# adamchang2000/DenseFusion

Measured on AMD Instinct MI355X. Metric: poses/sec (node) YCB-Video 1000 pts + 2 refine iters, higher is better.
Workload: dtype f32

## Files before the change

densefusion_amd/csrc/split_gemm.hip:

```cpp
#include "igemm.h"
#ifdef DF_DEV
#include <map>
#include <mutex>
#include <tuple>
#endif

namespace df {
namespace {

typedef __bf16 bf16x8 __attribute__((ext_vector_type(8)));
typedef __bf16 bf16x2 __attribute__((ext_vector_type(2)));
typedef float f32x16 __attribute__((ext_vector_type(16)));
typedef float f32x2 __attribute__((ext_vector_type(2)));

constexpr int SBM = 128, SBN = 128, SBK = 32;
constexpr int PLANE_BYTES = 128 * 64;

__device__ __forceinline__ void cut3(float a0, float a1, unsigned &hi, unsigned &mid, unsigned &lo) {
  const bf16x2 h = __builtin_convertvector(f32x2{a0, a1}, bf16x2);
  hi = __builtin_bit_cast(unsigned, h);
  const float r0 = a0 - __builtin_bit_cast(float, hi << 16), r1 = a1 - __builtin_bit_cast(float, hi & 0xFFFF0000u);
  const bf16x2 m = __builtin_convertvector(f32x2{r0, r1}, bf16x2);
  mid = __builtin_bit_cast(unsigned, m);
  const float s0 = r0 - __builtin_bit_cast(float, mid << 16), s1 = r1 - __builtin_bit_cast(float, mid & 0xFFFF0000u);
  const bf16x2 l = __builtin_convertvector(f32x2{s0, s1}, bf16x2);
  lo = __builtin_bit_cast(unsigned, l);
}

__global__ void cut_planes_kernel(const float *__restrict__ w, __bf16 *__restrict__ planes, long elems, long stride) {
  const long i = (long)blockIdx.x * blockDim.x + threadIdx.x;
  if (i >= elems) return;
  unsigned h, m, l;
  cut3(w[i], 0.f, h, m, l);
  unsigned short *pl = reinterpret_cast<unsigned short *>(planes);
  pl[i] = (unsigned short)h; pl[stride + i] = (unsigned short)m; pl[2 * stride + i] = (unsigned short)l;
}

struct SplitArgs {
  const float *in; const __bf16 *wpl; const float *bias; const float *res; const float *prelu; float *out; float *colsum;
  long M, wplane;
  int N, K, in_ld, in_coff, out_ld, out_coff, res_ld, res_coff, act, rows_per_group, rows_valid, bias_group_ld;
  long z_in_coff, z_wgt, z_bias, z_out_coff;
  int tiles_m, tiles_n;
  long cs_rows;
};

__device__ __forceinline__ int piece(int row, int slot) { return row * 64 + ((slot ^ ((row >> 2) & 3)) << 4); }

__device__ __forceinline__ void split_epilogue(const SplitArgs &a, const f32x16 (&acc)[2][2], int z, long row0, int wrow, int nb, int fr, int fh, long cs_row) {
  const float slope = a.act == ACT_PRELU ? a.prelu[0] : 0.f;
  float *out = a.out + z * a.z_out_coff + a.out_coff;
  const float *bias = a.bias ? a.bias + z * a.z_bias : nullptr;
  const float *gbias = bias && a.bias_group_ld > 0 ? bias + (row0 / a.rows_per_group) * a.bias_group_ld : nullptr;
  const int grp = a.rows_per_group > 0 ? (int)(row0 / a.rows_per_group) : 0;
  const long left = a.M - row0;
  const int valid = a.rows_per_group > 0 ? a.rows_valid - (int)(row0 - (long)grp * a.rows_per_group) : (1 << 30);
  const int limit = (int)(left < valid ? left : valid);
#pragma unroll
  for (int j = 0; j < 2; ++j) {
    const int n = nb + j * 32 + fr;
    const float b1 = gbias ? gbias[n] : bias ? bias[n] : 0.f;
    float csum = 0.f;
#pragma unroll
    for (int i = 0; i < 2; ++i) {
      const int tb = wrow + i * 32 + 4 * fh;
      const long mb = row0 + tb;
      float r[16];
      if (a.res) {
#pragma unroll
        for (int e = 0; e < 16; ++e) {
          long m = mb + (e & 3) + 8 * (e >> 2);
          m = m < a.M ? m : a.M - 1;
          r[e] = a.res[m * a.res_ld + a.res_coff + n];
        }
      }
#pragma unroll
      for (int e = 0; e < 16; ++e) {
        const int tr = tb + (e & 3) + 8 * (e >> 2);
        const long m = row0 + tr;
        float v = acc[i][j][e] + b1;
        if (a.res) v += r[e];
        if (a.act == ACT_RELU) v = v > 0.f ? v : 0.f;
        else if (a.act == ACT_PRELU) v = v > 0.f ? v : v * slope;
        if (a.out && m < a.M) out[m * a.out_ld + n] = v;
        csum += tr < limit ? v : 0.f;
      }
    }
    if (a.colsum && cs_row < a.cs_rows) {
      csum += __shfl_xor(csum, 32);
      if (fh == 0) a.colsum[((size_t)z * a.cs_rows + (size_t)cs_row) * a.N + n] = csum;
    }
  }
}

__global__ __launch_bounds__(256, 2) void gemm_split_bf16_kernel(const SplitArgs a) {
  __shared__ __attribute__((aligned(16))) unsigned char lds[6 * PLANE_BYTES];
  const int tid = threadIdx.x, lane = tid & 63, wave = tid >> 6;
  const int xcd = blockIdx.x & 7, seq = blockIdx.x >> 3;
  const int tm = (seq / a.tiles_n) * 8 + xcd, tn = seq % a.tiles_n;
  if (tm >= a.tiles_m) return;
  const int z = blockIdx.z;
  const long row0 = (long)tm * SBM;
  const int n0 = tn * SBN;
  const float *in = a.in + z * a.z_in_coff + a.in_coff;
  const __bf16 *wpl = a.wpl + z * a.z_wgt;

  const int srow0 = tid >> 2, srow1 = srow0 + 64, sslot = tid & 3;
  const int soff0 = piece(srow0, sslot), soff1 = piece(srow1, sslot);
  long r0 = row0 + srow0, r1 = row0 + srow1;
  r0 = r0 < a.M ? r0 : a.M - 1;
  r1 = r1 < a.M ? r1 : a.M - 1;
  const float *ag0 = in + r0 * a.in_ld + sslot * 8, *ag1 = in + r1 * a.in_ld + sslot * 8;
  const __bf16 *bg0 = wpl + (long)(n0 + srow0) * a.K + sslot * 8, *bg1 = wpl + (long)(n0 + srow1) * a.K + sslot * 8;
  float4 xa00, xa01, xa10, xa11, ya00, ya01, ya10, ya11;
  uint4 rb00, rb01, rb02, rb10, rb11, rb12;
#define SPLIT_FETCH_A(S, k0)                                                     \
  do {                                                                           \
    S##a00 = *reinterpret_cast<const float4 *>(ag0 + (k0));                      \
    S##a01 = *reinterpret_cast<const float4 *>(ag0 + (k0) + 4);                  \
    S##a10 = *reinterpret_cast<const float4 *>(ag1 + (k0));                      \
    S##a11 = *reinterpret_cast<const float4 *>(ag1 + (k0) + 4);                  \
  } while (0)
#define SPLIT_FETCH_B(k0)                                                        \
  do {                                                                           \
    rb00 = *reinterpret_cast<const uint4 *>(bg0 + (k0));                         \
    rb01 = *reinterpret_cast<const uint4 *>(bg0 + a.wplane + (k0));              \
    rb02 = *reinterpret_cast<const uint4 *>(bg0 + 2 * a.wplane + (k0));          \
    rb10 = *reinterpret_cast<const uint4 *>(bg1 + (k0));                         \
    rb11 = *reinterpret_cast<const uint4 *>(bg1 + a.wplane + (k0));              \
    rb12 = *reinterpret_cast<const uint4 *>(bg1 + 2 * a.wplane + (k0));          \
  } while (0)
#define SPLIT_STAGE1(x0, x1, off, b0, b1, b2)                                    \
  do {                                                                           \
    uint4 h, m, l;                                                               \
    cut3(x0.x, x0.y, h.x, m.x, l.x);                                             \
    cut3(x0.z, x0.w, h.y, m.y, l.y);                                             \
    cut3(x1.x, x1.y, h.z, m.z, l.z);                                             \
    cut3(x1.z, x1.w, h.w, m.w, l.w);                                             \
    *reinterpret_cast<uint4 *>(lds + (off)) = h;                                 \
    *reinterpret_cast<uint4 *>(lds + PLANE_BYTES + (off)) = m;                   \
    *reinterpret_cast<uint4 *>(lds + 2 * PLANE_BYTES + (off)) = l;               \
    *reinterpret_cast<uint4 *>(lds + 3 * PLANE_BYTES + (off)) = b0;              \
    *reinterpret_cast<uint4 *>(lds + 4 * PLANE_BYTES + (off)) = b1;              \
    *reinterpret_cast<uint4 *>(lds + 5 * PLANE_BYTES + (off)) = b2;              \
  } while (0)
#define SPLIT_STAGE(S)                                                           \
  do {                                                                           \
    SPLIT_STAGE1(S##a00, S##a01, soff0, rb00, rb01, rb02);                       \
    SPLIT_STAGE1(S##a10, S##a11, soff1, rb10, rb11, rb12);                       \
  } while (0)

  const int wr = wave >> 1, wc = wave & 1, fr = lane & 31, fh = lane >> 5;
  f32x16 acc[2][2];
#pragma unroll
  for (int i = 0; i < 2; ++i)
#pragma unroll
    for (int j = 0; j < 2; ++j)
#pragma unroll
      for (int e = 0; e < 16; ++e) acc[i][j][e] = 0.f;
  int offa[2][2], offb[2][2];
#pragma unroll
  for (int ks = 0; ks < 2; ++ks)
#pragma unroll
    for (int t = 0; t < 2; ++t) {
      offa[ks][t] = piece(wr * 64 + t * 32 + fr, ks * 2 + fh);
      offb[ks][t] = 3 * PLANE_BYTES + piece(wc * 64 + t * 32 + fr, ks * 2 + fh);
    }

#define SPLIT_COMPUTE()                                                                                   \
  _Pragma("unroll") for (int ks = 0; ks < 2; ++ks) {                                                      \
    bf16x8 fa[2][3], fb[2][3];                                                                            \
    _Pragma("unroll") for (int t = 0; t < 2; ++t)                                                         \
    _Pragma("unroll") for (int p = 0; p < 3; ++p) {                                                       \
      fa[t][p] = *reinterpret_cast<const bf16x8 *>(lds + p * PLANE_BYTES + offa[ks][t]);                  \
      fb[t][p] = *reinterpret_cast<const bf16x8 *>(lds + p * PLANE_BYTES + offb[ks][t]);                  \
    }                                                                                                     \
    _Pragma("unroll") for (int i = 0; i < 2; ++i)                                                         \
    _Pragma("unroll") for (int j = 0; j < 2; ++j) {                                                       \
      f32x16 c = acc[i][j];                                                        \
      c = __builtin_amdgcn_mfma_f32_32x32x16_bf16(fa[i][2], fb[j][0], c, 0, 0, 0);                        \
      c = __builtin_amdgcn_mfma_f32_32x32x16_bf16(fa[i][0], fb[j][2], c, 0, 0, 0);                        \
      c = __builtin_amdgcn_mfma_f32_32x32x16_bf16(fa[i][1], fb[j][1], c, 0, 0, 0);                        \
      c = __builtin_amdgcn_mfma_f32_32x32x16_bf16(fa[i][1], fb[j][0], c, 0, 0, 0);                        \
      c = __builtin_amdgcn_mfma_f32_32x32x16_bf16(fa[i][0], fb[j][1], c, 0, 0, 0);                        \
      c = __builtin_amdgcn_mfma_f32_32x32x16_bf16(fa[i][0], fb[j][0], c, 0, 0, 0);                        \
      acc[i][j] = c;                                                                                      \
    }                                                                                                     \
  }

  const int nk = a.K / SBK;
  SPLIT_FETCH_A(x, 0);
  SPLIT_FETCH_B(0);
  if (nk > 1) SPLIT_FETCH_A(y, SBK);
  SPLIT_STAGE(x);
  __syncthreads();
  for (int kt = 0; kt < nk; kt += 2) {
    if (kt + 1 < nk) SPLIT_FETCH_B((kt + 1) * SBK);
    if (kt + 2 < nk) SPLIT_FETCH_A(x, (kt + 2) * SBK);
    SPLIT_COMPUTE();
    if (kt + 1 >= nk) break;
    __syncthreads();
    SPLIT_STAGE(y);
    __syncthreads();
    if (kt + 2 < nk) SPLIT_FETCH_B((kt + 2) * SBK);
    if (kt + 3 < nk) SPLIT_FETCH_A(y, (kt + 3) * SBK);
    SPLIT_COMPUTE();
    if (kt + 2 >= nk) break;
    __syncthreads();
    SPLIT_STAGE(x);
    __syncthreads();
  }

  split_epilogue(a, acc, z, row0, wr * 64, n0 + wc * 64, fr, fh, (long)tm * 2 + wr);
}

constexpr int V2_APL = 256 * 64, V2_BPL = 128 * 64, V2_STAGE = 3 * V2_APL + 3 * V2_BPL;

__global__ __launch_bounds__(512, 1) void gemm_split_bf16_v2_kernel(const SplitArgs a) {
  extern __shared__ __attribute__((aligned(16))) unsigned char lds2[];
  const int tid = threadIdx.x, lane = tid & 63, wave = tid >> 6;
  const int xcd = blockIdx.x & 7, seq = blockIdx.x >> 3;
  const int tm = (seq / a.tiles_n) * 8 + xcd, tn = seq % a.tiles_n;
  if (tm >= a.tiles_m) return;
  const int z = blockIdx.z;
  const long row0 = (long)tm * 256;
  const int n0 = tn * SBN;
  const float *in = a.in + z * a.z_in_coff + a.in_coff;
  const __bf16 *wpl = a.wpl + z * a.z_wgt;

  const int srow0 = tid >> 2, srow1 = srow0 + 128, sslot = tid & 3;
  const int soff0 = piece(srow0, sslot), soff1 = piece(srow1, sslot);
  long r0 = row0 + srow0, r1 = row0 + srow1;
  r0 = r0 < a.M ? r0 : a.M - 1;
  r1 = r1 < a.M ? r1 : a.M - 1;
  const float *ag0 = in + r0 * a.in_ld + sslot * 8, *ag1 = in + r1 * a.in_ld + sslot * 8;
  const __bf16 *bg0 = wpl + (long)(n0 + srow0) * a.K + sslot * 8;
  float4 xa00, xa01, xa10, xa11, ya00, ya01, ya10, ya11;
  uint4 xb0, xb1, xb2, yb0, yb1, yb2;
#define V2_FETCH(S, k0)                                                          \
  do {                                                                           \
    S##a00 = *reinterpret_cast<const float4 *>(ag0 + (k0));                      \
    S##a01 = *reinterpret_cast<const float4 *>(ag0 + (k0) + 4);                  \
    S##a10 = *reinterpret_cast<const float4 *>(ag1 + (k0));                      \
    S##a11 = *reinterpret_cast<const float4 *>(ag1 + (k0) + 4);                  \
    S##b0 = *reinterpret_cast<const uint4 *>(bg0 + (k0));                        \
    S##b1 = *reinterpret_cast<const uint4 *>(bg0 + a.wplane + (k0));             \
    S##b2 = *reinterpret_cast<const uint4 *>(bg0 + 2 * a.wplane + (k0));         \
  } while (0)
#define V2_CUT(x0, x1, base, off)                                                \
  do {                                                                           \
    uint4 h, m, l;                                                               \
    cut3(x0.x, x0.y, h.x, m.x, l.x);                                             \
    cut3(x0.z, x0.w, h.y, m.y, l.y);                                             \
    cut3(x1.x, x1.y, h.z, m.z, l.z);                                             \
    cut3(x1.z, x1.w, h.w, m.w, l.w);                                             \
    *reinterpret_cast<uint4 *>((base) + (off)) = h;                              \
    *reinterpret_cast<uint4 *>((base) + V2_APL + (off)) = m;                     \
    *reinterpret_cast<uint4 *>((base) + 2 * V2_APL + (off)) = l;                 \
  } while (0)
#define V2_STAGE_TO(S, base)                                                     \
  do {                                                                           \
    V2_CUT(S##a00, S##a01, base, soff0);                                         \
    V2_CUT(S##a10, S##a11, base, soff1);                                         \
    *reinterpret_cast<uint4 *>((base) + 3 * V2_APL + soff0) = S##b0;             \
    *reinterpret_cast<uint4 *>((base) + 3 * V2_APL + V2_BPL + soff0) = S##b1;    \
    *reinterpret_cast<uint4 *>((base) + 3 * V2_APL + 2 * V2_BPL + soff0) = S##b2; \
  } while (0)

  const int wr = wave >> 1, wc = wave & 1, fr = lane & 31, fh = lane >> 5;
  f32x16 acc[2][2];
#pragma unroll
  for (int i = 0; i < 2; ++i)
#pragma unroll
    for (int j = 0; j < 2; ++j)
#pragma unroll
      for (int e = 0; e < 16; ++e) acc[i][j][e] = 0.f;
  int offa[2][2], offb[2][2];
#pragma unroll
  for (int ks = 0; ks < 2; ++ks)
#pragma unroll
    for (int t = 0; t < 2; ++t) {
      offa[ks][t] = piece(wr * 64 + t * 32 + fr, ks * 2 + fh);
      offb[ks][t] = 3 * V2_APL + piece(wc * 64 + t * 32 + fr, ks * 2 + fh);
    }
#define V2_COMPUTE(base)                                                                                  \
  _Pragma("unroll") for (int ks = 0; ks < 2; ++ks) {                                                      \
    bf16x8 fa[2][3], fb[2][3];                                                                            \
    _Pragma("unroll") for (int t = 0; t < 2; ++t)                                                         \
    _Pragma("unroll") for (int p = 0; p < 3; ++p) {                                                       \
      fa[t][p] = *reinterpret_cast<const bf16x8 *>((base) + p * V2_APL + offa[ks][t]);                    \
      fb[t][p] = *reinterpret_cast<const bf16x8 *>((base) + p * V2_BPL + offb[ks][t]);                    \
    }                                                                                                     \
    _Pragma("unroll") for (int q = 0; q < 6; ++q) {                                                       \
      constexpr int PA[6] = {2, 0, 1, 1, 0, 0}, PB[6] = {0, 2, 1, 0, 1, 0};                               \
      _Pragma("unroll") for (int i = 0; i < 2; ++i)                                                       \
      _Pragma("unroll") for (int j = 0; j < 2; ++j)                                                       \
        acc[i][j] = __builtin_amdgcn_mfma_f32_32x32x16_bf16(fa[i][PA[q]], fb[j][PB[q]], acc[i][j], 0, 0, 0); \
    }                                                                                                     \
  }
#define V2_BODY(FS, SS, kf, cur, nxt)                                            \
  do {                                                                           \
    V2_FETCH(FS, (kf));                                                          \
    V2_STAGE_TO(SS, nxt);                                                        \
    V2_COMPUTE(cur);                                                             \
    __builtin_amdgcn_sched_group_barrier(0x020, 7, 0);                           \
    __builtin_amdgcn_sched_group_barrier(0x100, 12, 0);                          \
    _Pragma("unroll") for (int g = 0; g < 48; ++g) {                             \
      __builtin_amdgcn_sched_group_barrier(0x008, 1, 0);                         \
      __builtin_amdgcn_sched_group_barrier(0x002, 2, 0);                         \
      if (g >= 8 && g < 32 && (g & 1) == 0) __builtin_amdgcn_sched_group_barrier(0x100, 1, 0); \
      if (g % 5 == 4) __builtin_amdgcn_sched_group_barrier(0x200, 1, 0);         \
    }                                                                            \
    __syncthreads();                                                             \
  } while (0)

  unsigned char *const st0 = lds2, *const st1 = lds2 + V2_STAGE;
  const int nk = a.K / SBK;
  const int klast = a.K - SBK;
  V2_FETCH(x, 0);
  V2_FETCH(y, SBK < klast ? SBK : klast);
  V2_STAGE_TO(x, st0);
  __syncthreads();
  int kt = 0;
  for (; kt + 1 < nk; kt += 2) {
    const int k2 = (kt + 2) * SBK, k3 = (kt + 3) * SBK;
    V2_BODY(x, y, k2 < klast ? k2 : klast, st0, st1);
    V2_BODY(y, x, k3 < klast ? k3 : klast, st1, st0);
  }
  if (nk & 1) { V2_COMPUTE(st0); }
  split_epilogue(a, acc, z, row0, wr * 64, n0 + wc * 64, fr, fh, (long)tm * 4 + wr);
}

#ifdef DF_DEV
std::mutex g_mu;
std::map<std::tuple<int, hipStream_t>, std::pair<__bf16 *, long>> g_scratch;

const __bf16 *scratch_planes(const float *w, long elems, hipStream_t st) {
  int dev = 0;
  (void)hipGetDevice(&dev);
  std::lock_guard<std::mutex> g(g_mu);
  auto &sc = g_scratch[std::make_tuple(dev, st)];
  if (sc.second < elems) {
    if (sc.first) (void)hipFree(sc.first);
    sc = {nullptr, 0};
    if (hipMalloc(reinterpret_cast<void **>(&sc.first), (size_t)elems * 3 * sizeof(__bf16)) != hipSuccess) return nullptr;
    sc.second = elems;
  }
  cut_weight_planes(w, sc.first, elems, elems, st);
  return sc.first;
}
#endif

}

int split_route(int N, int K, int epi) {
  if (N <= 0 || N % SBN != 0 || K % SBK != 0 || K < 384) return 0;
  return epi == GEMM_EPI_PLAIN || epi == GEMM_EPI_RESIDUAL || epi == GEMM_EPI_GROUPS;
}

int gemm_epi_kind(const ConvParams &p) {
  const bool groups = p.rows_per_group > 0 || p.bias_group_ld > 0 || p.colsum;
  if (p.res) return groups ? GEMM_EPI_OTHER : GEMM_EPI_RESIDUAL;
  return groups ? GEMM_EPI_GROUPS : GEMM_EPI_PLAIN;
}

void cut_weight_planes(const float *w, void *planes, long elems, long stride, hipStream_t st) {
  hipLaunchKernelGGL(cut_planes_kernel, dim3((unsigned)((elems + 255) / 256)), dim3(256), 0, st, w, reinterpret_cast<__bf16 *>(planes), elems, stride);
}

int try_split_gemm(const ConvParams &p, hipStream_t st) {
  static const bool off = dev_getenv("DF_GEMM_SPLIT_OFF") != nullptr;
  static const bool all = dev_getenv("DF_GEMM_SPLIT_BF16") != nullptr;
  static const bool verbose = dev_getenv("DF_GEMM_SPLIT_VERBOSE") != nullptr;
  if (off || p.splitk_ws || (!p.wpl && !all)) return 0;
  const long M = (long)p.B * p.OH * p.OW;
  const int K = p.Cin;
  const bool ok = p.KH == 1 && p.KW == 1 && p.stride == 1 && p.pad == 0 && p.up == 1 && p.H == p.OH && p.W == p.OW && (p.out || p.colsum) &&
                  p.Cout % SBN == 0 && K % SBK == 0 && K >= SBK && M >= 1 && gemm_epi_kind(p) != GEMM_EPI_OTHER &&
                  (p.rows_per_group == 0 ? p.bias_group_ld == 0 : p.rows_per_group % SBM == 0) && (p.z_wgt % 8) == 0;
  const bool take = ok && (all || split_route(p.Cout, K, gemm_epi_kind(p)));
  if (verbose) fprintf(stderr, "[df-split] M=%ld N=%d K=%d z%d -> %s\n", M, p.Cout, K, p.zcount, take ? "bf16 x 6" : "fp32");
  if (!take) {
    if (p.wpl && !all) return set_error(DF_ERR_ARG, "split gemm: routed launch M=%ld N=%d K=%d outside the kernels' cover", M, p.Cout, K);
    return 0;
  }
  const __bf16 *wpl = reinterpret_cast<const __bf16 *>(p.wpl);
  long wplane = p.wpl_stride;
#ifdef DF_DEV
  if (!wpl) {
    wplane = (long)(p.zcount - 1) * p.z_wgt + (long)p.Cout * K;
    wpl = scratch_planes(p.wgt, wplane, st);
    if (!wpl) return set_error(DF_ERR_LAUNCH, "split gemm: hipMalloc of the weight-plane scratch failed");
  }
#endif
  SplitArgs a{};
  a.in = p.in; a.wpl = wpl; a.bias = p.bias; a.res = p.res; a.prelu = p.prelu; a.out = p.out; a.colsum = p.colsum;
  a.M = M; a.wplane = wplane; a.N = p.Cout; a.K = K; a.in_ld = p.in_ld; a.in_coff = p.in_coff; a.out_ld = p.out_ld; a.out_coff = p.out_coff;
  a.res_ld = p.res_ld; a.res_coff = p.res_coff; a.act = p.act; a.rows_per_group = p.rows_per_group; a.rows_valid = p.rows_valid; a.bias_group_ld = p.bias_group_ld;
  a.z_in_coff = p.z_in_coff; a.z_wgt = p.z_wgt; a.z_bias = p.z_bias; a.z_out_coff = p.z_out_coff;
  a.cs_rows = ((M + 127) / 128) * 2;
  a.tiles_n = p.Cout / SBN;
  static const int variant = dev_getenv("DF_GEMM_SPLIT_V") ? atoi(dev_getenv("DF_GEMM_SPLIT_V")) : 2;
  const bool v2 = variant == 2 && K >= 384 && (p.rows_per_group == 0 || p.rows_per_group % 256 == 0);
  if (v2) {
    const int rc = raise_lds_limit(reinterpret_cast<const void *>(&gemm_split_bf16_v2_kernel), 2 * V2_STAGE);
    if (rc != DF_OK) return rc;
    a.tiles_m = (int)((M + 255) / 256);
    const unsigned grid = (unsigned)(((a.tiles_m + 7) / 8) * 8 * a.tiles_n);
    hipLaunchKernelGGL(gemm_split_bf16_v2_kernel, dim3(grid, 1, p.zcount), dim3(512), 2 * V2_STAGE, st, a);
  } else {
    a.tiles_m = (int)((M + SBM - 1) / SBM);
    const unsigned grid = (unsigned)(((a.tiles_m + 7) / 8) * 8 * a.tiles_n);
    hipLaunchKernelGGL(gemm_split_bf16_kernel, dim3(grid, 1, p.zcount), dim3(256), 0, st, a);
  }
  return 1;
}

}
```

Baseline: 9737.

## Add 256x256 split-bf16 GEMM kernel with LDS-staged vectorized epilogue

Adds a v3 split-bf16 GEMM that uses 256x256 output tiles with K steps of 16 and 32x32x16 MFMAs. It interleaves LDS reads, the fp32-to-three-bf16 splitting and LDS writes with MFMAs through sched_group_barrier. The epilogue stages each wave's results in LDS so it can issue float4 coalesced stores, with residual and activation applied on the vector path. The kernel is selected by default when Cout is a multiple of 256, pointers and strides allow 16-byte alignment, and the tile count reaches the CU count. The aim is more data reuse per block and fewer global store transactions, at the cost of larger LDS use (128KB), one block per CU and fewer tiles for small problems.

```diff
diff --git a/densefusion_amd/csrc/split_gemm.hip b/densefusion_amd/csrc/split_gemm.hip
--- a/densefusion_amd/csrc/split_gemm.hip
+++ b/densefusion_amd/csrc/split_gemm.hip
@@ -1,4 +1,6 @@
 #include "igemm.h"
+#include <atomic>
+#include <cstdint>
 #ifdef DF_DEV
 #include <map>
 #include <mutex>
@@ -91,6 +93,66 @@
       if (fh == 0) a.colsum[((size_t)z * a.cs_rows + (size_t)cs_row) * a.N + n] = csum;
     }
   }
+}
+
+__device__ __forceinline__ void split_epilogue_rows(const SplitArgs &a, const f32x16 (&acc)[2][2], int z, long row0, int wrow, int nb, int lane, long cs_row, float *blk) {
+  const int fr = lane & 31, fh = lane >> 5;
+  const float slope = a.act == ACT_PRELU ? a.prelu[0] : 0.f;
+  const float *bias = a.bias ? a.bias + z * a.z_bias : nullptr;
+  const float *gbias = bias && a.bias_group_ld > 0 ? bias + (row0 / a.rows_per_group) * a.bias_group_ld : nullptr;
+  const int grp = a.rows_per_group > 0 ? (int)(row0 / a.rows_per_group) : 0;
+  const long left = a.M - row0;
+  const int valid = a.rows_per_group > 0 ? a.rows_valid - (int)(row0 - (long)grp * a.rows_per_group) : (1 << 30);
+  const int limit = (int)(left < valid ? left : valid);
+#pragma unroll
+  for (int j = 0; j < 2; ++j) {
+    const int n = nb + j * 32 + fr;
+    const float b1 = gbias ? gbias[n] : bias ? bias[n] : 0.f;
+    float csum = 0.f;
+#pragma unroll
+    for (int i = 0; i < 2; ++i)
+#pragma unroll
+      for (int e = 0; e < 16; ++e) {
+        const int br = i * 32 + 4 * fh + (e & 3) + 8 * (e >> 2);
+        float v = acc[i][j][e] + b1;
+        if (!a.res) {
+          if (a.act == ACT_RELU) v = v > 0.f ? v : 0.f;
+          else if (a.act == ACT_PRELU) v = v > 0.f ? v : v * slope;
+        }
+        blk[br * 64 + j * 32 + fr] = v;
+        csum += wrow + br < limit ? v : 0.f;
+      }
+    if (a.colsum && cs_row < a.cs_rows) {
+      csum += __shfl_xor(csum, 32);
+      if (fh == 0) a.colsum[((size_t)z * a.cs_rows + (size_t)cs_row) * a.N + n] = csum;
+    }
+  }
+  if (!a.out) return;
+  __builtin_amdgcn_fence(__ATOMIC_RELEASE, "wavefront");
+  __builtin_amdgcn_wave_barrier();
+  __builtin_amdgcn_fence(__ATOMIC_ACQUIRE, "wavefront");
+  float *out = a.out + z * a.z_out_coff + a.out_coff;
+  const int c4 = (lane & 15) * 4;
+#pragma unroll 4
+  for (int it = 0; it < 16; ++it) {
+    const int br = it * 4 + (lane >> 4);
+    const long m = row0 + wrow + br;
+    float4 v = *reinterpret_cast<const float4 *>(blk + br * 64 + c4);
+    if (m < a.M) {
+      if (a.res) {
+        const float4 r = *reinterpret_cast<const float4 *>(a.res + m * a.res_ld + a.res_coff + nb + c4);
+        v.x += r.x; v.y += r.y; v.z += r.z; v.w += r.w;
+        if (a.act == ACT_RELU) {
+          v.x = v.x > 0.f ? v.x : 0.f; v.y = v.y > 0.f ? v.y : 0.f; v.z = v.z > 0.f ? v.z : 0.f; v.w = v.w > 0.f ? v.w : 0.f;
+        } else if (a.act == ACT_PRELU) {
+          v.x = v.x > 0.f ? v.x : v.x * slope; v.y = v.y > 0.f ? v.y : v.y * slope; v.z = v.z > 0.f ? v.z : v.z * slope; v.w = v.w > 0.f ? v.w : v.w * slope;
+        }
+      }
+      *reinterpret_cast<float4 *>(out + m * a.out_ld + nb + c4) = v;
+    }
+  }
+  __builtin_amdgcn_fence(__ATOMIC_RELEASE, "wavefront");
+  __builtin_amdgcn_wave_barrier();
 }
 
 __global__ __launch_bounds__(256, 2) void gemm_split_bf16_kernel(const SplitArgs a) {
@@ -331,6 +393,146 @@
   split_epilogue(a, acc, z, row0, wr * 64, n0 + wc * 64, fr, fh, (long)tm * 4 + wr);
 }
 
+constexpr int V3_PL = 256 * 32, V3_STAGE = 6 * V3_PL;
+constexpr int V3_LDS = 8 * 64 * 64 * 4;
+
+__device__ __forceinline__ int piece16(int row, int half) { return row * 32 + ((half ^ ((row >> 3) & 1)) << 4); }
+
+__global__ __launch_bounds__(512, 1) void gemm_split_bf16_v3_kernel(const SplitArgs a) {
+  extern __shared__ __attribute__((aligned(16))) unsigned char lds3[];
+  const int tid = threadIdx.x, lane = tid & 63, wave = tid >> 6;
+  const int xcd = blockIdx.x & 7, seq = blockIdx.x >> 3;
+  const int tm = (seq / a.tiles_n) * 8 + xcd, tn = seq % a.tiles_n;
+  if (tm >= a.tiles_m) return;
+  const int z = blockIdx.z;
+  const long row0 = (long)tm * 256;
+  const int n0 = tn * 256;
+  const float *in = a.in + z * a.z_in_coff + a.in_coff;
+  const __bf16 *wpl = a.wpl + z * a.z_wgt;
+
+  const int srow = tid >> 1, shalf = tid & 1;
+  const int soff = piece16(srow, shalf);
+  long r = row0 + srow;
+  r = r < a.M ? r : a.M - 1;
+  const float *ag = in + r * a.in_ld + shalf * 8;
+  const __bf16 *bg = wpl + (long)(n0 + srow) * a.K + shalf * 8;
+  float4 xa0, xa1, ya0, ya1;
+  uint4 b0, b1, b2;
+#define V3_FETCH_A(S, k0)                                                        \
+  do {                                                                           \
+    S##a0 = *reinterpret_cast<const float4 *>(ag + (k0));                        \
+    S##a1 = *reinterpret_cast<const float4 *>(ag + (k0) + 4);                    \
+  } while (0)
+#define V3_FETCH_B(k0)                                                           \
+  do {                                                                           \
+    b0 = *reinterpret_cast<const uint4 *>(bg + (k0));                            \
+    b1 = *reinterpret_cast<const uint4 *>(bg + a.wplane + (k0));                 \
+    b2 = *reinterpret_cast<const uint4 *>(bg + 2 * a.wplane + (k0));             \
+  } while (0)
+#define V3_PIN(v) asm volatile("" : "+v"(v.x), "+v"(v.y), "+v"(v.z), "+v"(v.w))
+#define V3_CUT0(S) do { V3_PIN(S##a0); cut3(S##a0.x, S##a0.y, ch.x, cm.x, cl.x); cut3(S##a0.z, S##a0.w, ch.y, cm.y, cl.y); } while (0)
+#define V3_CUT1(S) do { V3_PIN(S##a1); cut3(S##a1.x, S##a1.y, ch.z, cm.z, cl.z); cut3(S##a1.z, S##a1.w, ch.w, cm.w, cl.w); } while (0)
+#define V3_WRITE_A(base)                                                         \
+  do {                                                                           \
+    *reinterpret_cast<uint4 *>((base) + soff) = ch;                              \
+    *reinterpret_cast<uint4 *>((base) + V3_PL + soff) = cm;                      \
+    *reinterpret_cast<uint4 *>((base) + 2 * V3_PL + soff) = cl;                  \
+  } while (0)
+#define V3_WRITE_B(base)                                                         \
+  do {                                                                           \
+    *reinterpret_cast<uint4 *>((base) + 3 * V3_PL + soff) = b0;                  \
+    *reinterpret_cast<uint4 *>((base) + 4 * V3_PL + soff) = b1;                  \
+    *reinterpret_cast<uint4 *>((base) + 5 * V3_PL + soff) = b2;                  \
+  } while (0)
+
+  const int wr = wave >> 2, wc = wave & 3, fr = lane & 31, fh = lane >> 5;
+  f32x16 acc[2][2][2];
+#pragma unroll
+  for (int h = 0; h < 2; ++h)
+#pragma unroll
+    for (int i = 0; i < 2; ++i)
+#pragma unroll
+      for (int j = 0; j < 2; ++j)
+#pragma unroll
+        for (int e = 0; e < 16; ++e) acc[h][i][j][e] = 0.f;
+  const int offa = piece16(wr * 128 + fr, fh), offb = 3 * V3_PL + piece16(wc * 64 + fr, fh);
+#define V3_PA(q) ((q) == 0 ? 2 : (q) == 2 || (q) == 3 ? 1 : 0)
+#define V3_PB(q) ((q) == 1 ? 2 : (q) == 2 || (q) == 4 ? 1 : 0)
+#define V3_READ(base, q)                                                                                  \
+  do {                                                                                                    \
+    _Pragma("unroll") for (int t = 0; t < 4; ++t)                                                         \
+      fa[t][V3_PA(q)] = *reinterpret_cast<const bf16x8 *>((base) + V3_PA(q) * V3_PL + offa + t * 1024);   \
+    _Pragma("unroll") for (int t = 0; t < 2; ++t)                                                         \
+      fb[t][V3_PB(q)] = *reinterpret_cast<const bf16x8 *>((base) + V3_PB(q) * V3_PL + offb + t * 1024);   \
+  } while (0)
+#define V3_MFMA(q)                                                                                        \
+  do {                                                                                                    \
+    _Pragma("unroll") for (int i = 0; i < 4; ++i)                                                         \
+    _Pragma("unroll") for (int j = 0; j < 2; ++j)                                                         \
+      acc[i >> 1][i & 1][j] = __builtin_amdgcn_mfma_f32_32x32x16_bf16(fa[i][V3_PA(q)], fb[j][V3_PB(q)], acc[i >> 1][i & 1][j], 0, 0, 0); \
+  } while (0)
+#define V3_WEAVE(n, mask, cnt)                                                   \
+  do {                                                                           \
+    _Pragma("unroll") for (int g = 0; g < (n); ++g) {                            \
+      __builtin_amdgcn_sched_group_barrier(0x008, 1, 0);                         \
+      __builtin_amdgcn_sched_group_barrier(mask, cnt, 0);                        \
+    }                                                                            \
+    __builtin_amdgcn_sched_barrier(0);                                           \
+  } while (0)
+#define V3_BODY(FS, SS, ka, kb, cur, nxt)                                        \
+  do {                                                                           \
+    bf16x8 fa[4][3], fb[2][3];                                                   \
+    uint4 ch, cm, cl;                                                            \
+    V3_FETCH_B(kb);                                                              \
+    V3_FETCH_A(FS, ka);                                                          \
+    V3_READ(cur, 0);                                                             \
+    __builtin_amdgcn_sched_barrier(0);                                           \
+    V3_READ(cur, 1);                                                             \
+    V3_MFMA(0);                                                                  \
+    V3_WEAVE(6, 0x100, 1);                                                       \
+    V3_READ(cur, 2);                                                             \
+    V3_MFMA(1);                                                                  \
+    V3_WEAVE(6, 0x100, 1);                                                       \
+    V3_CUT0(SS);                                                                 \
+    V3_MFMA(2);                                                                  \
+    V3_WEAVE(8, 0x002, 3);                                                       \
+    V3_CUT1(SS);                                                                 \
+    V3_MFMA(3);                                                                  \
+    V3_WEAVE(8, 0x002, 3);                                                       \
+    V3_WRITE_A(nxt);                                                             \
+    V3_MFMA(4);                                                                  \
+    V3_WEAVE(3, 0x200, 1);                                                       \
+    V3_WRITE_B(nxt);                                                             \
+    V3_MFMA(5);                                                                  \
+    V3_WEAVE(3, 0x200, 1);                                                       \
+    __syncthreads();                                                             \
+  } while (0)
+
+  unsigned char *const st0 = lds3, *const st1 = lds3 + V3_STAGE;
+  const int nk = a.K / 16;
+  const int klast = a.K - 16;
+  V3_FETCH_B(0);
+  V3_FETCH_A(x, 0);
+  V3_FETCH_A(y, 16);
+  {
+    uint4 ch, cm, cl;
+    V3_CUT0(x);
+    V3_CUT1(x);
+    V3_WRITE_A(st0);
+    V3_WRITE_B(st0);
+  }
+  __syncthreads();
+  for (int s = 0; s < nk; s += 2) {
+    const int k1 = (s + 1) * 16, k2 = (s + 2) * 16, k3 = (s + 3) * 16;
+    V3_BODY(x, y, k2 < klast ? k2 : klast, k1, st0, st1);
+    V3_BODY(y, x, k3 < klast ? k3 : klast, k2 < klast ? k2 : klast, st1, st0);
+  }
+  const int cs0 = tm * 4 + wr * 2;
+  float *const blk = reinterpret_cast<float *>(lds3) + wave * (64 * 64);
+  split_epilogue_rows(a, acc[0], z, row0, wr * 128, n0 + wc * 64, lane, (long)cs0, blk);
+  split_epilogue_rows(a, acc[1], z, row0, wr * 128 + 64, n0 + wc * 64, lane, (long)cs0 + 1, blk);
+}
+
 #ifdef DF_DEV
 std::mutex g_mu;
 std::map<std::tuple<int, hipStream_t>, std::pair<__bf16 *, long>> g_scratch;
@@ -366,6 +568,19 @@
 
 void cut_weight_planes(const float *w, void *planes, long elems, long stride, hipStream_t st) {
   hipLaunchKernelGGL(cut_planes_kernel, dim3((unsigned)((elems + 255) / 256)), dim3(256), 0, st, w, reinterpret_cast<__bf16 *>(planes), elems, stride);
+}
+
+static int compute_units() {
+  static std::atomic<int> cus[64];
+  int dev = 0;
+  (void)hipGetDevice(&dev);
+  if (dev < 0 || dev >= 64) return 256;
+  int n = cus[dev].load(std::memory_order_relaxed);
+  if (n == 0) {
+    if (hipDeviceGetAttribute(&n, hipDeviceAttributeMultiprocessorCount, dev) != hipSuccess || n <= 0) n = 256;
+    cus[dev].store(n, std::memory_order_relaxed);
+  }
+  return n;
 }
 
 int try_split_gemm(const ConvParams &p, hipStream_t st) {
@@ -400,9 +615,21 @@
   a.z_in_coff = p.z_in_coff; a.z_wgt = p.z_wgt; a.z_bias = p.z_bias; a.z_out_coff = p.z_out_coff;
   a.cs_rows = ((M + 127) / 128) * 2;
   a.tiles_n = p.Cout / SBN;
-  static const int variant = dev_getenv("DF_GEMM_SPLIT_V") ? atoi(dev_getenv("DF_GEMM_SPLIT_V")) : 2;
-  const bool v2 = variant == 2 && K >= 384 && (p.rows_per_group == 0 || p.rows_per_group % 256 == 0);
-  if (v2) {
+  static const int variant = dev_getenv("DF_GEMM_SPLIT_V") ? atoi(dev_getenv("DF_GEMM_SPLIT_V")) : 3;
+  const bool v2 = variant >= 2 && K >= 384 && (p.rows_per_group == 0 || p.rows_per_group % 256 == 0);
+  const long tiles3 = ((M + 255) / 256) * (p.Cout / 256) * p.zcount;
+  const bool rows16 = (!p.out || (reinterpret_cast<uintptr_t>(p.out) % 16 == 0 && p.out_ld % 4 == 0 && p.out_coff % 4 == 0 && p.z_out_coff % 4 == 0)) &&
+                      (!p.res || (reinterpret_cast<uintptr_t>(p.res) % 16 == 0 && p.res_ld % 4 == 0 && p.res_coff % 4 == 0));
+  const bool v3 = v2 && variant >= 3 && p.Cout % 256 == 0 && rows16 && tiles3 >= compute_units();
+  if (verbose) fprintf(stderr, "[df-split]   form %s\n", v3 ? "256x256" : v2 ? "256x128" : "128x128");
+  if (v3) {
+    const int rc = raise_lds_limit(reinterpret_cast<const void *>(&gemm_split_bf16_v3_kernel), V3_LDS);
+    if (rc != DF_OK) return rc;
+    a.tiles_m = (int)((M + 255) / 256);
+    a.tiles_n = p.Cout / 256;
+    const unsigned grid = (unsigned)(((a.tiles_m + 7) / 8) * 8 * a.tiles_n);
+    hipLaunchKernelGGL(gemm_split_bf16_v3_kernel, dim3(grid, 1, p.zcount), dim3(512), V3_LDS, st, a);
+  } else if (v2) {
     const int rc = raise_lds_limit(reinterpret_cast<const void *>(&gemm_split_bf16_v2_kernel), 2 * V2_STAGE);
     if (rc != DF_OK) return rc;
     a.tiles_m = (int)((M + 255) / 256);
```

New measurement: 10470 (median of 6 runs). 1.08x the previous value.
